# yweweler/single-speaker-tts

Measured on AMD Instinct MI355X. Metric: mel-frames/sec (end-to-end text->waveform incl. 60-iter Griffin-Lim, 64-utt LJ-Speech-shaped batch per GPU), higher is better.
Workload: dtype f32

## Files before the change

### single-speaker-tts_amd/csrc/api_internal.h

```cpp
#pragma once
#include <cmath>
#include <cstdio>
#include <cstring>
#include <memory>
#include <mutex>
#include <string>
#include <utility>
#include <vector>
#include "decoder.h"
#include "griffin_lim.h"
#include "tts_common.h"
#include <algorithm>
#include <map>

namespace tts_api {
using namespace tts;


extern thread_local std::string g_create_error;

struct ManifestEntry {
    std::string name;
    std::vector<int64_t> shape;
    size_t numel() const {
// ... 9 lines not shown
    const float* proj_wt[2];
    const float* proj_b[2];
    const float* proj_scale[2];
    const float* proj_shift[2];
    const float* lifter_wt;
    const float* lifter_b;
    std::vector<const float*> hw_wt, hw_b;
    const float* gru_in_wt;
    const float* gru_in_b;
    const float* gru_rec;
};

enum Stage { ST_ENCODER = 0, ST_DECODER, ST_POSTNET, ST_DENORM, ST_GL_ITER, ST_GL_FINAL, ST_DEBUG_GEMM, ST_EVAL_LOSS, ST_FEATURES, ST_COUNT };
extern const char* const kStageNames[ST_COUNT];

struct ProfSpan {
    hipEvent_t a, b;
    int stage;
    int64_t launches;
};


}
using namespace tts_api;

struct tts_handle_s {
    tts_config_t cfg;
    int device = 0;
    hipStream_t stream = nullptr;
    bool own_stream = false;
    std::string err;
    int use_graph = 0;
    int fused_tail = 1;
    bool tail_configured = false;
    int profile = 0;
    int pipeline = 1;
    int reserve_cus = 32;
    int hold_lds_kb = 64;
    hipStream_t aux = nullptr;
    int* hold_flags = nullptr;
    hipEvent_t ev_aux = nullptr;
    unsigned call_count = 0;
    hipStream_t front = nullptr;
    hipStream_t encs = nullptr;
    int enc_stream = 1;
    hipEvent_t ev_enc_ready[2] = {nullptr, nullptr};
    hipEvent_t ev_dec_done[2] = {nullptr, nullptr};
    hipEvent_t ev_gap[2] = {nullptr, nullptr};
    bool enc_ready_pending[2] = {false, false}, dec_done_pending[2] = {false, false}, gap_pending[2] = {false, false};
    hipEvent_t ev_front_done = nullptr;
    hipEvent_t ev_post_done[2] = {nullptr, nullptr};
    bool post_pending[2] = {false, false};
    bool gl_wide_used[2] = {false, false};
    hipEvent_t ev_gl_done[2] = {nullptr, nullptr};
    bool gl_pending[2] = {false, false};
    bool front_pending = false;
    hipEvent_t ev_serial_done = nullptr;
    bool serial_pending = false;
    unsigned syn_calls = 0;
    int syn_shape[3] = {0, 0, 0};
    int last_enc_ahead = -1;
    bool in_synthesize = false;
    int persistent_decoder = 1;
    int pd_ws = 1;
    bool ws_configured = false;
    int gl_pair = 3;
// ... 176 lines not shown
        if (!h->profile) return;
        ProfSpan s{};
        if (hipEventCreate(&s.a) != hipSuccess || hipEventCreate(&s.b) != hipSuccess) return;
        s.stage = stage;
        s.launches = launches;
        hipEventRecord(s.a, h->stream);
        h->spans.push_back(s);
        idx = (int)h->spans.size() - 1;
    }
    ~ProfScope() {
        if (idx >= 0) hipEventRecord(h->spans[idx].b, h->stream);
    }
};

struct SynthScope {
    tts_handle_t h;
    explicit SynthScope(tts_handle_t h_) : h(h_) { h->in_synthesize = true; }
    ~SynthScope() { h->in_synthesize = false; }
};

int fail(tts_handle_t h, int code, const std::string& msg);
void build_manifest(tts_handle_t h);
int check_status(tts_handle_t h);
int sync_all(tts_handle_t h);
int graph_quiesce(tts_handle_t h);
int graph_drop(tts_handle_t h);
int ws_get(tts_handle_t h, const char* name, size_t bytes, void** out);
void prof_collect(tts_handle_t h);
void feat_release(tts_handle_t h);
GemmGroup dense_group(const float* A, int lda, const float* Wt, const float* bias, float* C, int ldc, int M, int N, int K, int act);
GemmGroup conv_group(const float* A, int Cin, int ktaps, int T, const float* Wt, const float* bias, const float* scale, const float* shift, float* C, int ldc, int coff, int M, int N, int act, int pool);
int run_single(tts_handle_t h, const GemmGroup& g);
bool graph_runtime_ok(int* have);
int run_cbhg(tts_handle_t h, const CbhgWeights& w, const char* tag, const float* x, int B, int T, float* out, int64_t* launches);
int check_ready(tts_handle_t h);
int gl_tables(tts_handle_t h);
int device_cus(tts_handle_t h);
int stft_prepare(tts_handle_t h, int n, int win, int hop, int n_fft);
int stft_run(tts_handle_t h, const float* wav, int B, int n, int n_fft, int win, int hop, float2** out, int* Tf_out);
int gl_fp(int n_fft);
bool gl_is_streaming(int n_fft, int win, int hop);
int glg_twiddles(tts_handle_t h, int n_fft, const float2** out);
int glg_prepare(tts_handle_t h, int T, int win, int hop, int n_fft);
int gl_run_generic(tts_handle_t h, const float* mag_int, const float* init_ft, uint64_t seed, int B, int T, int n_iter, int win, int hop, int n_fft, float* wav, float* mse, bool peak_normalize);
int gl_prepare(tts_handle_t h, int T, int win, int hop, int n_fft);
int gl_run(tts_handle_t h, const float* mag_int, const float* init_ft, uint64_t seed, int B, int T, int n_iter, int win, int hop, int n_fft, float* wav, float* mse, bool peak_normalize = false, bool under_reservation = false, float2* const* phase_pair = nullptr, bool phase_ready = false, int wide_from = -1);
int standalone_begin(tts_handle_t h);
int standalone_end(tts_handle_t h);
int encoder_impl(tts_handle_t h, const int32_t* ids, int B, int Ts, float* memory);
int pd_kernel_for(tts_handle_t h, int B, int Ts, int budget);
int pd_choice(tts_handle_t h, int B, int Ts, int budget, bool pipelined);
int attention_keys(tts_handle_t h, const float* memory, int B, int Ts, float* keys);
int decoder_impl(tts_handle_t h, const float* memory, int B, int Ts, int n_steps, float* mel, float* alignments);
int postnet_impl(tts_handle_t h, const float* mel, int B, int T, float* linear, float* mag, float ref_db, float max_db, float power, int* db_flag = nullptr);
bool denorm_can_assert(float ref_db, float max_db);
int denorm_flag_arm(tts_handle_t h, int** flag);
int denorm_flag_read(tts_handle_t h);
int gl_wide_from(tts_handle_t h, int B, int Ts, int n_steps, int T, int n_iter);

}
```

### single-speaker-tts_amd/csrc/api_stages.hip

```cpp
#include "api_internal.h"

namespace tts_api {


int run_cbhg(tts_handle_t h, const CbhgWeights& w, const char* tag, const float* x, int B, int T, float* out,
             int64_t* launches) {
    const tts_config_t& c = h->cfg;
    const int M = B * T;
    const int NB = w.n_banks, NF = w.n_filters;
    const int U = c.n_highway_units, H = c.n_gru_units;
    const std::string t(tag);
    WS(h, (t + ".bank").c_str(), float, (size_t)M * NB * NF, bank);
    WS(h, (t + ".p1").c_str(), float, (size_t)M * w.proj_filters[0], p1);
    WS(h, (t + ".p2").c_str(), float, (size_t)M * w.proj_filters[1], p2);
    WS(h, (t + ".hw0").c_str(), float, (size_t)M * U, hw0);
    WS(h, (t + ".hw1").c_str(), float, (size_t)M * U, hw1);
    WS(h, (t + ".xproj").c_str(), float, (size_t)M * 6 * H, xproj);

    for (int k0 = 0; k0 < NB; k0 += TTS_GEMM_MAX_GROUPS) {
        GemmBatch b;
        std::memset(&b, 0, sizeof(b));
        const int ng = std::min(TTS_GEMM_MAX_GROUPS, NB - k0);
        for (int i = 0; i < ng; ++i) {
            const int k = k0 + ng - 1 - i;
            b.g[i] = conv_group(x, w.c_in, k + 1, T, w.bank_wt[k], w.bank_b[k], w.bank_scale[k], w.bank_shift[k], bank,
                                NB * NF, k * NF, M, NF, ACT_RELU, 0);
        }
        HIPCHK(h, launch_gemm(h->stream, b, ng));
        ++*launches;
    }
    {
        GemmGroup g = conv_group(bank, NB * NF, 3, T, w.proj_wt[0], w.proj_b[0], w.proj_scale[0], w.proj_shift[0], p1,
                                 w.proj_filters[0], 0, M, w.proj_filters[0], ACT_RELU, 1);
        const int slices = gemm_splitk_slices(g.K);
        if (slices > 1) {
            WS(h, (t + ".splitk").c_str(), float, (size_t)slices * M * g.N, part);
            HIPCHK(h, launch_gemm_splitk(h->stream, g, slices, part));
            ++*launches;
        } else {
            int rc = run_single(h, g);
            if (rc) return rc;
        }
        ++*launches;
    }
    {
        GemmGroup g = conv_group(p1, w.proj_filters[0], 3, T, w.proj_wt[1], w.proj_b[1], w.proj_scale[1],
                                 w.proj_shift[1], p2, w.proj_filters[1], 0, M, w.proj_filters[1], ACT_NONE, 0);
        g.R = x;
        g.ldr = w.c_in;
        int rc = run_single(h, g);
        if (rc) return rc;
        ++*launches;
    }
    if (h->fused_tail && cbhg_tail_supports(w.proj_filters[1], U, H, (int)w.hw_wt.size(), M)) {
        if (!h->tail_configured) {
            HIPCHK(h, cbhg_tail_configure());
            h->tail_configured = true;
        }
        CbhgTailParams tp;
        std::memset(&tp, 0, sizeof(tp));
        tp.X = p2; tp.ldx = w.proj_filters[1]; tp.c_in = w.proj_filters[1];
        tp.lifter_wt = w.lifter_wt; tp.lifter_b = w.lifter_b;
        tp.n_hw = (int)w.hw_wt.size();
        for (int l = 0; l < tp.n_hw; ++l) { tp.hw_wt[l] = w.hw_wt[l]; tp.hw_b[l] = w.hw_b[l]; }
        tp.gru_wt = w.gru_in_wt; tp.gru_b = w.gru_in_b;
        tp.hw_out = hw0; tp.xproj = xproj; tp.M = M;
        HIPCHK(h, launch_cbhg_tail(h->stream, tp));
        ++*launches;
    } else {
        {
            int rc = run_single(h, dense_group(p2, w.proj_filters[1], w.lifter_wt, w.lifter_b, hw0, U, M, U,
                                               w.proj_filters[1], ACT_RELU));
            if (rc) return rc;
            ++*launches;
        }
        float* cur = hw0;
        float* nxt = hw1;
        for (size_t l = 0; l < w.hw_wt.size(); ++l) {
            GemmGroup g = dense_group(cur, U, w.hw_wt[l], w.hw_b[l], nxt, U, M, 2 * U, U, ACT_NONE);
            g.epi = EPI_HIGHWAY;
            int rc = run_single(h, g);
            if (rc) return rc;
            ++*launches;
            std::swap(cur, nxt);
        }
        {
            int rc = run_single(h, dense_group(cur, U, w.gru_in_wt, w.gru_in_b, xproj, 6 * H, M, 6 * H, U, ACT_NONE));
            if (rc) return rc;
            ++*launches;
        }
    }
    HIPCHK(h, launch_bigru(h->stream, xproj, 6 * H, w.gru_rec, out, B, T, H, c.force_cudnn));
    ++*launches;
    return TTS_OK;
}


int check_ready(tts_handle_t h) {
    if (!h) return TTS_ERR_INVALID;
// ... 373 lines not shown
        if (h->dec_done_pending[i]) HIPCHK(h, hipStreamWaitEvent(h->stream, h->ev_dec_done[i], 0));
    }
    return TTS_OK;
}

int standalone_end(tts_handle_t h) {
    if (h->in_synthesize || !h->front) return TTS_OK;
    if (!h->ev_serial_done) HIPCHK(h, hipEventCreateWithFlags(&h->ev_serial_done, hipEventDisableTiming));
    HIPCHK(h, hipEventRecord(h->ev_serial_done, h->stream));
    h->serial_pending = true;
    return TTS_OK;
}

int encoder_impl(tts_handle_t h, const int32_t* ids, int B, int Ts, float* memory) {
    int rc = TTS_OK;
    const tts_config_t& c = h->cfg;
    const int M = B * Ts;
    WS(h, "enc.pre1", float, (size_t)M * c.enc_prenet_units[0], pre1);
    WS(h, "enc.pre2", float, (size_t)M * c.enc_prenet_units[1], pre2);
    int64_t launches = 0;
    ProfScope ps(h, ST_ENCODER, 0);
    {
        GemmGroup g = dense_group(h->embedding, c.embedding_size, h->enc_pre_wt[0], h->enc_pre_b[0], pre1,
                                  c.enc_prenet_units[0], M, c.enc_prenet_units[0], c.embedding_size, ACT_RELU);
        g.gather = ids;
        g.gather_rows = c.vocabulary_size;
        if ((rc = run_single(h, g))) return rc;
    }
    if ((rc = run_single(h, dense_group(pre1, c.enc_prenet_units[0], h->enc_pre_wt[1], h->enc_pre_b[1], pre2,
                                        c.enc_prenet_units[1], M, c.enc_prenet_units[1], c.enc_prenet_units[0],
                                        ACT_RELU))))
        return rc;
    launches += 2;
    if ((rc = run_cbhg(h, h->enc, "enc", pre2, B, Ts, memory, &launches))) return rc;
    if (ps.idx >= 0) h->spans[ps.idx].launches = launches;
    return TTS_OK;
}


int pd_kernel_for(tts_handle_t h, int B, int Ts, int budget) {
    const int cudnn = h->cfg.force_cudnn;
    if (h->pd_ws && decoder_ws_supports(h->dec, cudnn, B, Ts) && decoder_ws_workgroups(B) <= budget) return 2;
    if (decoder_persistent_supports(h->dec, cudnn, B, Ts) && decoder_persistent_workgroups(B) <= budget) return 1;
    return 0;
}


int pd_choice(tts_handle_t h, int B, int Ts, int budget, bool pipelined) {
    if (h->persistent_decoder <= 0) return 0;
    const int k = pd_kernel_for(h, B, Ts, budget);
    if (h->persistent_decoder >= 2) return k;
    if (k == 2) return 2;
    if (k == 1) return (pipelined && B > 48) ? 1 : 0;
    return 0;
}


int attention_keys(tts_handle_t h, const float* memory, int B, int Ts, float* keys) {
    const int A = h->cfg.n_attention_units, mem = 2 * h->cfg.n_gru_units;
    return run_single(h, dense_group(memory, mem, h->mem_wt, nullptr, keys, A, B * Ts, A, mem, ACT_NONE));
}

int decoder_impl(tts_handle_t h, const float* memory, int B, int Ts, int n_steps, float* mel, float* alignments) {
    int rc = TTS_OK;
    const tts_config_t& c = h->cfg;
    if (h->dec.local_d > 0 && Ts < 2 * h->dec.local_d + 1)
        return fail(h, TTS_ERR_UNSUPPORTED,
// ... 131 lines not shown
        if (defer_proj) {
            h->pending_proj = proj;
            h->has_pending_proj = true;
        } else if ((rc = run_single(h, proj))) {
            return rc;
        }
    }
    if (predictive) {
        int flag = 0;
        HIPCHK(h, hipMemcpyAsync(&flag, sc.err_flag, sizeof(int), hipMemcpyDeviceToHost, h->stream));
        HIPCHK(h, hipStreamSynchronize(h->stream));
        if (flag)
            return fail(h, TTS_ERR_UNSUPPORTED,
                        "LocalLuongAttention (predictive): a predicted attention window leaves the memory; the "
                        "reference pads such windows inconsistently and fails there too");
    }
    return TTS_OK;
}


int postnet_impl(tts_handle_t h, const float* mel, int B, int T, float* linear, float* mag, float ref_db,
                        float max_db, float power, int* db_flag) {
    int rc = check_ready(h);
    if (rc) return rc;
    if (!mel || (!linear && !mag) || B < 1 || T < 1) return fail(h, TTS_ERR_INVALID, "postnet_forward: bad arguments");
    const tts_config_t& c = h->cfg;
    const int M = B * T, H2 = 2 * c.n_gru_units, F = 1 + c.n_fft / 2;
    int64_t launches = 0;
    ProfScope ps(h, ST_POSTNET, 0);
    const float* dense_in = mel;
    int dense_k = c.n_mels;
    if (c.apply_post_processing) {
        WS(h, "post.gru", float, (size_t)M * H2, gru);
        if ((rc = run_cbhg(h, h->post, "post", mel, B, T, gru, &launches))) return rc;
        dense_in = gru;
        dense_k = H2;
    }
    GemmGroup g = dense_group(dense_in, dense_k, h->dense_wt, h->dense_b, linear, F, M, F, dense_k, ACT_NONE);
    if (mag) {
        g.C2 = mag;
        g.ldc2 = gl_fp(c.n_fft);
        g.N2 = gl_fp(c.n_fft);
        g.d_ref = ref_db;
        g.d_range = std::fabs(ref_db) + std::fabs(max_db);
        g.d_pow = power;
        g.d_flag = db_flag;
    }
    if ((rc = run_single(h, g))) return rc;
    ++launches;
    if (ps.idx >= 0) h->spans[ps.idx].launches = launches;
    return TTS_OK;
}


bool denorm_can_assert(float ref_db, float max_db) {
    return ref_db - (std::fabs(ref_db) + std::fabs(max_db)) < -100.0f;
}

int denorm_flag_arm(tts_handle_t h, int** flag) {
    if (!h->an.flag) HIPCHK(h, hipMalloc(&h->an.flag, sizeof(int)));
    HIPCHK(h, hipMemsetAsync(h->an.flag, 0, sizeof(int), h->stream));
    *flag = h->an.flag;
    return TTS_OK;
}

int denorm_flag_read(tts_handle_t h) {
    int flag = 0;
// ... 278 lines not shown
```

### single-speaker-tts_amd/csrc/cbhg_tail.hip

```cpp
#include "tts_common.h"

namespace tts {

#define CT_BM 128
#define CT_U 128
#define CT_XLD (CT_U + 4)
#define CT_BK 32
#define CT_BLD (CT_BK + 4)
#define CT_BN 256
#define CT_THREADS 512

#define CT_AIMG (3 * CT_BM * 64)
#define CT_BIMG (3 * CT_BN * 64)
size_t cbhg_tail_lds_bytes() { return (size_t)CT_BM * CT_XLD * sizeof(float) + CT_AIMG + CT_BIMG; }
typedef __bf16 ct_bf16x8_t __attribute__((ext_vector_type(8)));
__device__ __forceinline__ void ct_split3(float x, unsigned& h, unsigned& m, unsigned& l) {
    h = __float_as_uint(x);
    const float r1 = x - __uint_as_float(h & 0xFFFF0000u);
    m = __float_as_uint(r1);
    const float r2 = r1 - __uint_as_float(m & 0xFFFF0000u);
    l = __float_as_uint(r2);
}
__device__ __forceinline__ unsigned ct_pack_hi(unsigned a, unsigned b) { return __builtin_amdgcn_perm(b, a, 0x07060302u); }
__device__ __forceinline__ void ct_store_split4(unsigned char* img, int rows, int row, int kq, float4 v) {
    unsigned h[4], m[4], l[4];
    ct_split3(v.x, h[0], m[0], l[0]);
    ct_split3(v.y, h[1], m[1], l[1]);
    ct_split3(v.z, h[2], m[2], l[2]);
    ct_split3(v.w, h[3], m[3], l[3]);
    const int off = (row * 4 + ((kq >> 1) ^ ((row >> 2) & 3))) * 16 + (kq & 1) * 8;
    *reinterpret_cast<uint2*>(img + off) = make_uint2(ct_pack_hi(h[0], h[1]), ct_pack_hi(h[2], h[3]));
    *reinterpret_cast<uint2*>(img + rows * 64 + off) = make_uint2(ct_pack_hi(m[0], m[1]), ct_pack_hi(m[2], m[3]));
    *reinterpret_cast<uint2*>(img + 2 * rows * 64 + off) = make_uint2(ct_pack_hi(l[0], l[1]), ct_pack_hi(l[2], l[3]));
}

bool cbhg_tail_supports(int c_in, int units, int gru_units, int n_hw, long long M) {
    return units == CT_U && gru_units == 128 && c_in >= 4 && c_in <= CT_U && c_in % 4 == 0 && n_hw >= 0 && n_hw <= CBHG_TAIL_MAX_HW &&
           M >= 1 && (M + CT_BM) * 3 * CT_BN * (long long)sizeof(float) < 0xFFFFFFF0ll;
}

__global__ __launch_bounds__(CT_THREADS) void cbhg_tail_kernel(CbhgTailParams p) {
    extern __shared__ __attribute__((aligned(16))) float lds[];
    float* Xs = lds;
    unsigned char* Ai = reinterpret_cast<unsigned char*>(lds + CT_BM * CT_XLD);
    unsigned char* Bi = Ai + CT_AIMG;
    const int tid = threadIdx.x, lane = tid & 63, wave = tid >> 6;
    const int wm = wave & 1, wn = wave >> 1;
    const int li = lane & 31, lh = lane >> 5;
    const int m0 = blockIdx.x * CT_BM;
    const int M = p.M;

    {
        const __amdgpu_buffer_rsrc_t rs = __builtin_amdgcn_make_buffer_rsrc(const_cast<float*>(p.X), 0, (int)0xFFFFFFF0u, 0x00020000);
#pragma unroll
        for (int i = 0; i < (CT_BM * (CT_U / 4)) / CT_THREADS; ++i) {
            const int idx = tid + CT_THREADS * i;
            const int row = idx >> 5, c4 = idx & 31;
            const bool ok = m0 + row < M && 4 * c4 < p.c_in;
            const unsigned off = ok ? (unsigned)((size_t)(m0 + row) * p.ldx + 4 * c4) * 4u : 0xFFFFFFFFu;
            const float4 v = __builtin_bit_cast(float4, __builtin_amdgcn_raw_buffer_load_b128(rs, (int)off, 0, 0));
            *reinterpret_cast<float4*>(&Xs[row * CT_XLD + 4 * c4]) = v;
        }
    }

    const int n_jobs = 1 + p.n_hw + 3;
    const int kq = tid & 7;
    float4 rb[4];
    auto job_w = [&](int j) -> const float* {
        return j == 0 ? p.lifter_wt : (j <= p.n_hw ? p.hw_wt[j - 1] : p.gru_wt + (size_t)(j - 1 - p.n_hw) * CT_BN * CT_U);
    };
    auto job_k = [&](int j) { return j == 0 ? p.c_in : CT_U; };
    auto job_n = [&](int j) { return j == 0 ? CT_U : CT_BN; };
    auto load_chunk = [&](int j, int kc) {
        const __amdgpu_buffer_rsrc_t rs = __builtin_amdgcn_make_buffer_rsrc(const_cast<float*>(job_w(j)), 0, (int)0xFFFFFFF0u, 0x00020000);
        const int K = job_k(j), N = job_n(j);
        const int kk = kc * CT_BK + 4 * kq;
#pragma unroll
        for (int i = 0; i < 4; ++i) {
            const int row = (tid >> 3) + 64 * i;
            const bool ok = row < N && kk < K;
            rb[i] = __builtin_bit_cast(float4, __builtin_amdgcn_raw_buffer_load_b128(rs, ok ? (int)((unsigned)(row * K + kk) * 4u) : -1, 0, 0));
        }
    };
    auto stage_chunk = [&](int kc) {
#pragma unroll
        for (int i = 0; i < 4; ++i) ct_store_split4(Bi, CT_BN, (tid >> 3) + 64 * i, kq, rb[i]);
#pragma unroll
        for (int i = 0; i < 2; ++i) {
            const int row = (tid >> 3) + 64 * i;
            ct_store_split4(Ai, CT_BM, row, kq, *reinterpret_cast<const float4*>(&Xs[row * CT_XLD + kc * CT_BK + 4 * kq]));
        }
    };

    const __amdgpu_buffer_rsrc_t xp_rs = __builtin_amdgcn_make_buffer_rsrc(
        p.xproj, 0, (int)(unsigned)((size_t)M * 3 * CT_BN * sizeof(float) < 0xFFFFFFF0ull ? (size_t)M * 3 * CT_BN * sizeof(float) : 0xFFFFFFF0ull), 0x00020000);
    const __amdgpu_buffer_rsrc_t hw_rs = __builtin_amdgcn_make_buffer_rsrc(
        p.hw_out, 0, p.hw_out ? (int)(unsigned)((size_t)M * CT_U * sizeof(float)) : 0, 0x00020000);
    const int row_l = wm * 64 + 4 * lh;

    f32x16 acc[2][2];
    load_chunk(0, 0);
    for (int j = 0; j < n_jobs; ++j) {
        const int nch = (job_k(j) + CT_BK - 1) / CT_BK;
        const bool live = 64 * wn < job_n(j);
#pragma unroll
        for (int a = 0; a < 2; ++a)
#pragma unroll
            for (int b = 0; b < 2; ++b)
#pragma unroll
                for (int r = 0; r < 16; ++r) acc[a][b][r] = 0.f;
        for (int kc = 0; kc < nch; ++kc) {
            __syncthreads();
            stage_chunk(kc);
            __syncthreads();
            if (kc + 1 < nch) load_chunk(j, kc + 1);
            else if (j + 1 < n_jobs) load_chunk(j + 1, 0);
            if (live) {
#pragma unroll
                for (int q = 0; q < 2; ++q) {
                    const int ch = 2 * q + lh;
                    uint4 fa[2][3];
#pragma unroll
                    for (int tm = 0; tm < 2; ++tm) {
                        const int row = wm * 64 + tm * 32 + li;
                        const int off = (row * 4 + (ch ^ ((row >> 2) & 3))) * 16;
#pragma unroll
                        for (int sp = 0; sp < 3; ++sp) fa[tm][sp] = *reinterpret_cast<const uint4*>(Ai + sp * CT_BM * 64 + off);
                    }
#pragma unroll
                    for (int tn = 0; tn < 2; ++tn) {
                        const int row = wn * 64 + tn * 32 + li;
                        const int off = (row * 4 + (ch ^ ((row >> 2) & 3))) * 16;
                        uint4 fb[3];
#pragma unroll
                        for (int sp = 0; sp < 3; ++sp) fb[sp] = *reinterpret_cast<const uint4*>(Bi + sp * CT_BN * 64 + off);
#pragma unroll
                        for (int tm = 0; tm < 2; ++tm) {
#define CT_MMA(SA, SB)                                                                                                   \
                            acc[tm][tn] = __builtin_amdgcn_mfma_f32_32x32x16_bf16(__builtin_bit_cast(ct_bf16x8_t, fa[tm][SA]), \
                                                                                  __builtin_bit_cast(ct_bf16x8_t, fb[SB]), acc[tm][tn], 0, 0, 0);
                            CT_MMA(0, 2) CT_MMA(2, 0) CT_MMA(1, 1) CT_MMA(0, 1) CT_MMA(1, 0) CT_MMA(0, 0)
#undef CT_MMA
                        }
                    }
                }
            }
        }

        if (j == 0) {
            if (live) {
#pragma unroll
                for (int tn = 0; tn < 2; ++tn) {
                    const float b = p.lifter_b[wn * 64 + tn * 32 + li];
#pragma unroll
                    for (int tm = 0; tm < 2; ++tm)
#pragma unroll
                        for (int r = 0; r < 16; ++r) acc[tm][tn][r] = fmaxf(acc[tm][tn][r] + b, 0.f);
                }
            }
            __syncthreads();
            if (live) {
#pragma unroll
                for (int tn = 0; tn < 2; ++tn)
#pragma unroll
                    for (int tm = 0; tm < 2; ++tm)
#pragma unroll
                        for (int r = 0; r < 16; ++r) {
                            const int ro = tm * 32 + (r & 3) + 8 * (r >> 2);
                            Xs[(row_l + ro) * CT_XLD + wn * 64 + tn * 32 + li] = acc[tm][tn][r];
                        }
            }
        } else if (j <= p.n_hw) {
            const int unit = wn * 32 + li;
            const float bh = p.hw_b[j - 1][wn * 64 + li], bt = p.hw_b[j - 1][wn * 64 + 32 + li];
#pragma unroll
            for (int tm = 0; tm < 2; ++tm)
#pragma unroll
                for (int r = 0; r < 16; ++r) {
                    const int ro = tm * 32 + (r & 3) + 8 * (r >> 2);
                    const float hh = fmaxf(acc[tm][0][r] + bh, 0.f);
                    const float tt = sigmoidf_(acc[tm][1][r] + bt);
                    const float x = Xs[(row_l + ro) * CT_XLD + unit];
// ... 63 lines not shown
```

### single-speaker-tts_amd/csrc/tts_common.h

```cpp
#pragma once
#include <hip/hip_runtime.h>
#include <stdint.h>
#include <stddef.h>
#include <map>
#include <string>
#include <vector>

#include "../../include/sstts_hip.h"

namespace tts {

typedef float f32x4 __attribute__((ext_vector_type(4)));
typedef float f32x16 __attribute__((ext_vector_type(16)));

enum Act { ACT_NONE = 0, ACT_RELU = 1, ACT_SIGMOID = 2, ACT_TANH = 3 };
enum Epi { EPI_STD = 0, EPI_HIGHWAY = 1 };

__device__ __forceinline__ float sigmoidf_(float x) { return __builtin_amdgcn_rcpf(1.0f + __expf(-x)); }
__device__ __forceinline__ double wave_sum_f64(double v) {
#pragma unroll
    for (int o = 32; o > 0; o >>= 1) v += __shfl_xor(v, o);
    return v;
}
__device__ __forceinline__ void split_f64(double v, float* hi, float* lo) {
// ... 38 lines not shown
    const float* R;
    float* C;
    int M, N, K;
    int lda, T, Cin, padl, pool;
    int ldc, coff, ldr;
    int act, epi;
    float* C2;
    int ldc2, N2;
    float d_ref, d_range, d_pow;
    int* d_flag;
    int kt0, kt1;
};
#define TTS_GEMM_MAX_GROUPS 16
struct GemmBatch {
    GemmGroup g[TTS_GEMM_MAX_GROUPS];
};
hipError_t launch_gemm(hipStream_t s, const GemmBatch& b, int n_groups);
hipError_t launch_gemm_splitk(hipStream_t s, const GemmGroup& g, int slices, float* partial);
int gemm_splitk_slices(int K);

hipError_t launch_bigru(hipStream_t s, const float* xproj, int xld, const float* wrec, float* out,
                        int B, int T, int H, int cudnn);
size_t bigru_wrec_floats(int H, int cudnn);

#define CBHG_TAIL_MAX_HW 8
struct CbhgTailParams {
    const float* X; int ldx; int c_in;
    const float* lifter_wt; const float* lifter_b;
    const float* hw_wt[CBHG_TAIL_MAX_HW]; const float* hw_b[CBHG_TAIL_MAX_HW]; int n_hw;
    const float* gru_wt; const float* gru_b;
    float* hw_out;
    float* xproj;
    int M;
};
bool cbhg_tail_supports(int c_in, int units, int gru_units, int n_hw, long long M);
hipError_t cbhg_tail_configure();
hipError_t launch_cbhg_tail(hipStream_t s, const CbhgTailParams& p);

hipError_t cu_hold_configure();
hipError_t launch_cu_hold(hipStream_t s, int n_cus, const int* flag, double timeout_ms, int lds_kb = 64);

size_t eval_loss_partial_count(int B, int T, int n_mels, int F);
hipError_t launch_eval_loss(hipStream_t s, const float* mel_t, const float* mel_o, const float* lin_t, const float* lin_o, int B,
                            int T, int n_mels, int F, int max_blocks, double* partial, double* sums, float* losses);

struct DevBuf {
    void* p = nullptr;
    size_t bytes = 0;
};

}
```

### single-speaker-tts_amd/csrc/api_handle.hip

```cpp
#include "api_internal.h"

namespace tts_api {
thread_local std::string g_create_error;
const char* const kStageNames[ST_COUNT] = {"encoder", "decoder", "postnet", "denorm", "gl_iter", "gl_final", "debug_gemm", "eval_loss", "features"};
}

namespace tts_api {


int fail(tts_handle_t h, int code, const std::string& msg) {
    if (h) h->err = msg;
    else g_create_error = msg;
    return code;
}


const char* kAtt = "decoder2/decoder/output_projection_wrapper/multi_rnn_cell/cell_0/attention_wrapper";

const char* kMrc = "decoder2/decoder/output_projection_wrapper/multi_rnn_cell";


std::string bn_name(int i) {
    return i == 0 ? std::string("batch_normalization") : "batch_normalization_" + std::to_string(i);
}
// ... 621 lines not shown
    h->gl_pending[0] = h->gl_pending[1] = false;
    h->gl_wide_used[0] = h->gl_wide_used[1] = false;
    {
        int rc = graph_drop(h);
        if (rc) return rc;
    }
    if (h->own_stream) hipStreamDestroy(h->stream);
    if (s) {
        h->stream = reinterpret_cast<hipStream_t>(s);
        h->own_stream = false;
    } else {
        HIPCHK(h, hipStreamCreate(&h->stream));
        h->own_stream = true;
    }
    return TTS_OK;
}


int tts_set_option(tts_handle_t h, const char* key, int value) {
    DeviceScope dev_scope(h);
    if (!h || !key) return TTS_ERR_INVALID;
    if (!std::strcmp(key, "use_graph")) {
        int have = 0;
        if (value && !(value == 2 && h->debug_hooks) && !graph_runtime_ok(&have))
            return fail(h, TTS_ERR_UNSUPPORTED,
                        "use_graph: this process runs the library on HIP runtime " + std::to_string(have) + ", older than the " +
                        std::to_string(HIP_VERSION) + " it was built with (a libamdhip64 loaded before the library, e.g. the one "
                        "PyTorch bundles); hipGraph replays of the decoder are wrong there (csrc/api_internal.h, `use_graph`) -- the "
                        "launches are enqueued directly instead");
        h->use_graph = value;
    }
    else if (!std::strcmp(key, "profile")) h->profile = value;
    else if (!std::strcmp(key, "fused_tail")) h->fused_tail = value;
    else if (!std::strcmp(key, "persistent_decoder")) {
        if (value != h->persistent_decoder) {
            int rc = sync_all(h);
            if (rc) return rc;
        }
        h->persistent_decoder = value;
    }
    else if (!std::strcmp(key, "gl_pair")) h->gl_pair = value;
    else if (!std::strcmp(key, "gl_wide_from")) h->gl_wide = value < -2 ? -2 : value;
    else if (!std::strcmp(key, "pd_ws")) {
        if (value != h->pd_ws) {
            int rc = sync_all(h);
            if (rc) return rc;
        }
        h->pd_ws = value;
    }
    else if (!std::strcmp(key, "enc_stream")) {
        int rc = sync_all(h);
        if (rc) return rc;
        h->enc_stream = value;
    }
    else if (!std::strcmp(key, "debug_hooks")) h->debug_hooks = value;
    else if (!std::strcmp(key, "pd_debug_delay") || !std::strcmp(key, "gl_runs") || !std::strcmp(key, "gl_run_len") ||
             !std::strcmp(key, "timeline") || !std::strcmp(key, "gl_workers") || !std::strcmp(key, "pd_rows")) {
        if (!h->debug_hooks && value != 0)
            return fail(h, TTS_ERR_INVALID, std::string(key) + ": a test hook; set the option \"debug_hooks\" to 1 on this handle first");
        if (!std::strcmp(key, "pd_debug_delay")) h->pd_debug_delay = value;
        else if (!std::strcmp(key, "gl_runs")) h->gl_runs = value;
        else if (!std::strcmp(key, "gl_run_len")) h->gl_run_len = value;
        else if (!std::strcmp(key, "gl_workers")) h->gl_workers = value;
        else if (!std::strcmp(key, "pd_rows")) h->pd_rows = value;
        else h->timeline = value;
    }
// ... 327 lines not shown
```

Before: 4.391 million.

## Fold second CBHG projection conv and residual into fused tail kernel prologue

For the post-net CBHG, the second projection conv (3-tap over p1, with bias, batchnorm scale/shift and the residual add of the input) is computed inside the fused tail kernel as an extra GEMM job that writes straight into shared memory. This removes one kernel launch and the global write and re-read of the p2 intermediate. The encoder keeps the old path via keep_p2. The tail kernel becomes more complex and gains extra registers, and the prologue loads p1 rows per tap through buffer loads.

```diff
diff --git a/single-speaker-tts_amd/csrc/api_internal.h b/single-speaker-tts_amd/csrc/api_internal.h
--- a/single-speaker-tts_amd/csrc/api_internal.h
+++ b/single-speaker-tts_amd/csrc/api_internal.h
@@ -307,7 +307,8 @@
 GemmGroup conv_group(const float* A, int Cin, int ktaps, int T, const float* Wt, const float* bias, const float* scale, const float* shift, float* C, int ldc, int coff, int M, int N, int act, int pool);
 int run_single(tts_handle_t h, const GemmGroup& g);
 bool graph_runtime_ok(int* have);
-int run_cbhg(tts_handle_t h, const CbhgWeights& w, const char* tag, const float* x, int B, int T, float* out, int64_t* launches);
+int run_cbhg(tts_handle_t h, const CbhgWeights& w, const char* tag, const float* x, int B, int T, float* out, int64_t* launches,
+             bool keep_p2);
 int check_ready(tts_handle_t h);
 int gl_tables(tts_handle_t h);
 int device_cus(tts_handle_t h);
diff --git a/single-speaker-tts_amd/csrc/api_stages.hip b/single-speaker-tts_amd/csrc/api_stages.hip
--- a/single-speaker-tts_amd/csrc/api_stages.hip
+++ b/single-speaker-tts_amd/csrc/api_stages.hip
@@ -4,7 +4,7 @@
 
 
 int run_cbhg(tts_handle_t h, const CbhgWeights& w, const char* tag, const float* x, int B, int T, float* out,
-             int64_t* launches) {
+             int64_t* launches, bool keep_p2) {
     const tts_config_t& c = h->cfg;
     const int M = B * T;
     const int NB = w.n_banks, NF = w.n_filters;
@@ -43,7 +43,9 @@
         }
         ++*launches;
     }
-    {
+    const bool tail = h->fused_tail && cbhg_tail_supports(w.proj_filters[1], U, H, (int)w.hw_wt.size(), M);
+    const bool fold = tail && h->fused_tail != 2 && !keep_p2 && cbhg_tail_prologue_supports(w.proj_filters[0], w.proj_filters[1], M);
+    if (!fold) {
         GemmGroup g = conv_group(p1, w.proj_filters[0], 3, T, w.proj_wt[1], w.proj_b[1], w.proj_scale[1],
                                  w.proj_shift[1], p2, w.proj_filters[1], 0, M, w.proj_filters[1], ACT_NONE, 0);
         g.R = x;
@@ -52,7 +54,7 @@
         if (rc) return rc;
         ++*launches;
     }
-    if (h->fused_tail && cbhg_tail_supports(w.proj_filters[1], U, H, (int)w.hw_wt.size(), M)) {
+    if (tail) {
         if (!h->tail_configured) {
             HIPCHK(h, cbhg_tail_configure());
             h->tail_configured = true;
@@ -65,6 +67,12 @@
         for (int l = 0; l < tp.n_hw; ++l) { tp.hw_wt[l] = w.hw_wt[l]; tp.hw_b[l] = w.hw_b[l]; }
         tp.gru_wt = w.gru_in_wt; tp.gru_b = w.gru_in_b;
         tp.hw_out = hw0; tp.xproj = xproj; tp.M = M;
+        if (fold) {
+            tp.X = nullptr;
+            tp.p1 = p1; tp.p1_c = w.proj_filters[0]; tp.T = T;
+            tp.p2_wt = w.proj_wt[1]; tp.p2_b = w.proj_b[1]; tp.p2_scale = w.proj_scale[1]; tp.p2_shift = w.proj_shift[1];
+            tp.R = x; tp.ldr = w.c_in;
+        }
         HIPCHK(h, launch_cbhg_tail(h->stream, tp));
         ++*launches;
     } else {
@@ -504,7 +512,7 @@
                                         ACT_RELU))))
         return rc;
     launches += 2;
-    if ((rc = run_cbhg(h, h->enc, "enc", pre2, B, Ts, memory, &launches))) return rc;
+    if ((rc = run_cbhg(h, h->enc, "enc", pre2, B, Ts, memory, &launches, true))) return rc;
     if (ps.idx >= 0) h->spans[ps.idx].launches = launches;
     return TTS_OK;
 }
@@ -702,7 +710,7 @@
     int dense_k = c.n_mels;
     if (c.apply_post_processing) {
         WS(h, "post.gru", float, (size_t)M * H2, gru);
-        if ((rc = run_cbhg(h, h->post, "post", mel, B, T, gru, &launches))) return rc;
+        if ((rc = run_cbhg(h, h->post, "post", mel, B, T, gru, &launches, false))) return rc;
         dense_in = gru;
         dense_k = H2;
     }
diff --git a/single-speaker-tts_amd/csrc/cbhg_tail.hip b/single-speaker-tts_amd/csrc/cbhg_tail.hip
--- a/single-speaker-tts_amd/csrc/cbhg_tail.hip
+++ b/single-speaker-tts_amd/csrc/cbhg_tail.hip
@@ -34,6 +34,12 @@
     *reinterpret_cast<uint2*>(img + 2 * rows * 64 + off) = make_uint2(ct_pack_hi(l[0], l[1]), ct_pack_hi(l[2], l[3]));
 }
 
+bool cbhg_tail_prologue_supports(int p1_c, int c_in, long long M) {
+    return p1_c >= CT_BK && p1_c % CT_BK == 0 && c_in >= 4 && c_in <= CT_U && c_in % 4 == 0 &&
+           (M + CT_BM) * p1_c * (long long)sizeof(float) < 0xFFFFFFF0ll && (M + CT_BM) * CT_U * (long long)sizeof(float) < 0xFFFFFFF0ll &&
+           (long long)c_in * 3 * p1_c * (long long)sizeof(float) < 0xFFFFFFF0ll;
+}
+
 bool cbhg_tail_supports(int c_in, int units, int gru_units, int n_hw, long long M) {
     return units == CT_U && gru_units == 128 && c_in >= 4 && c_in <= CT_U && c_in % 4 == 0 && n_hw >= 0 && n_hw <= CBHG_TAIL_MAX_HW &&
            M >= 1 && (M + CT_BM) * 3 * CT_BN * (long long)sizeof(float) < 0xFFFFFFF0ll;
@@ -50,7 +56,8 @@
     const int m0 = blockIdx.x * CT_BM;
     const int M = p.M;
 
-    {
+    const bool pro = p.p1 != nullptr;
+    if (!pro) {
         const __amdgpu_buffer_rsrc_t rs = __builtin_amdgcn_make_buffer_rsrc(const_cast<float*>(p.X), 0, (int)0xFFFFFFF0u, 0x00020000);
 #pragma unroll
         for (int i = 0; i < (CT_BM * (CT_U / 4)) / CT_THREADS; ++i) {
@@ -63,32 +70,59 @@
         }
     }
 
+    const int j_first = pro ? -1 : 0;
     const int n_jobs = 1 + p.n_hw + 3;
     const int kq = tid & 7;
     float4 rb[4];
+    float4 ra[2];
     auto job_w = [&](int j) -> const float* {
-        return j == 0 ? p.lifter_wt : (j <= p.n_hw ? p.hw_wt[j - 1] : p.gru_wt + (size_t)(j - 1 - p.n_hw) * CT_BN * CT_U);
+        return j < 0 ? p.p2_wt : j == 0 ? p.lifter_wt : (j <= p.n_hw ? p.hw_wt[j - 1] : p.gru_wt + (size_t)(j - 1 - p.n_hw) * CT_BN * CT_U);
     };
-    auto job_k = [&](int j) { return j == 0 ? p.c_in : CT_U; };
-    auto job_n = [&](int j) { return j == 0 ? CT_U : CT_BN; };
+    auto job_k = [&](int j) { return j < 0 ? 3 * p.p1_c : j == 0 ? p.c_in : CT_U; };
+    auto job_n = [&](int j) { return j < 0 ? p.c_in : j == 0 ? CT_U : CT_BN; };
+    int pro_t[2] = {-1, -1};
+    if (pro) {
+#pragma unroll
+        for (int i = 0; i < 2; ++i) {
+            const int m = m0 + (tid >> 3) + 64 * i;
+            pro_t[i] = m < M ? m % p.T : -1;
+        }
+    }
+    auto chunk_k0 = [&](int j, int kc) { return j < 0 ? (kc % 3) * p.p1_c + (kc / 3) * CT_BK : kc * CT_BK; };
     auto load_chunk = [&](int j, int kc) {
         const __amdgpu_buffer_rsrc_t rs = __builtin_amdgcn_make_buffer_rsrc(const_cast<float*>(job_w(j)), 0, (int)0xFFFFFFF0u, 0x00020000);
         const int K = job_k(j), N = job_n(j);
-        const int kk = kc * CT_BK + 4 * kq;
+        const int kk = chunk_k0(j, kc) + 4 * kq;
 #pragma unroll
         for (int i = 0; i < 4; ++i) {
+            if (i >= 2 && N <= 128) break;
             const int row = (tid >> 3) + 64 * i;
             const bool ok = row < N && kk < K;
             rb[i] = __builtin_bit_cast(float4, __builtin_amdgcn_raw_buffer_load_b128(rs, ok ? (int)((unsigned)(row * K + kk) * 4u) : -1, 0, 0));
         }
+        if (j < 0) {
+            const __amdgpu_buffer_rsrc_t ps = __builtin_amdgcn_make_buffer_rsrc(const_cast<float*>(p.p1), 0, (int)0xFFFFFFF0u, 0x00020000);
+            const int tap = kc % 3, ch = (kc / 3) * CT_BK + 4 * kq;
+#pragma unroll
+            for (int i = 0; i < 2; ++i) {
+                const int ts = pro_t[i] - 1 + tap;
+                const bool ok = pro_t[i] >= 0 && ts >= 0 && ts < p.T;
+                const int src = m0 + (tid >> 3) + 64 * i - 1 + tap;
+                ra[i] = __builtin_bit_cast(float4, __builtin_amdgcn_raw_buffer_load_b128(
+                                                       ps, ok ? (int)((unsigned)(src * p.p1_c + ch) * 4u) : -1, 0, 0));
+            }
+        }
     };
-    auto stage_chunk = [&](int kc) {
-#pragma unroll
-        for (int i = 0; i < 4; ++i) ct_store_split4(Bi, CT_BN, (tid >> 3) + 64 * i, kq, rb[i]);
+    auto stage_chunk = [&](int j, int kc) {
+#pragma unroll
+        for (int i = 0; i < 4; ++i) {
+            if (i >= 2 && job_n(j) <= 128) break;
+            ct_store_split4(Bi, CT_BN, (tid >> 3) + 64 * i, kq, rb[i]);
+        }
 #pragma unroll
         for (int i = 0; i < 2; ++i) {
             const int row = (tid >> 3) + 64 * i;
-            ct_store_split4(Ai, CT_BM, row, kq, *reinterpret_cast<const float4*>(&Xs[row * CT_XLD + kc * CT_BK + 4 * kq]));
+            ct_store_split4(Ai, CT_BM, row, kq, j < 0 ? ra[i] : *reinterpret_cast<const float4*>(&Xs[row * CT_XLD + kc * CT_BK + 4 * kq]));
         }
     };
 
@@ -99,8 +133,8 @@
     const int row_l = wm * 64 + 4 * lh;
 
     f32x16 acc[2][2];
-    load_chunk(0, 0);
-    for (int j = 0; j < n_jobs; ++j) {
+    load_chunk(j_first, 0);
+    for (int j = j_first; j < n_jobs; ++j) {
         const int nch = (job_k(j) + CT_BK - 1) / CT_BK;
         const bool live = 64 * wn < job_n(j);
 #pragma unroll
@@ -111,7 +145,7 @@
                 for (int r = 0; r < 16; ++r) acc[a][b][r] = 0.f;
         for (int kc = 0; kc < nch; ++kc) {
             __syncthreads();
-            stage_chunk(kc);
+            stage_chunk(j, kc);
             __syncthreads();
             if (kc + 1 < nch) load_chunk(j, kc + 1);
             else if (j + 1 < n_jobs) load_chunk(j + 1, 0);
@@ -147,7 +181,41 @@
             }
         }
 
-        if (j == 0) {
+        if (j < 0) {
+            if (live) {
+#pragma unroll
+                for (int tn = 0; tn < 2; ++tn) {
+                    const int c = wn * 64 + tn * 32 + li;
+                    const bool cok = c < p.c_in;
+                    const float b = cok ? p.p2_b[c] : 0.f;
+                    const float sc = cok && p.p2_scale ? p.p2_scale[c] : 1.f;
+                    const float sh = cok && p.p2_scale ? p.p2_shift[c] : 0.f;
+#pragma unroll
+                    for (int tm = 0; tm < 2; ++tm)
+#pragma unroll
+                        for (int r = 0; r < 16; ++r) {
+                            const int ro = tm * 32 + (r & 3) + 8 * (r >> 2);
+                            float v = acc[tm][tn][r] + b;
+                            v = v * sc + sh;
+                            Xs[(row_l + ro) * CT_XLD + c] = v;
+                        }
+                }
+            }
+            __syncthreads();
+            const __amdgpu_buffer_rsrc_t rs = __builtin_amdgcn_make_buffer_rsrc(const_cast<float*>(p.R), 0, (int)0xFFFFFFF0u, 0x00020000);
+#pragma unroll 1
+            for (int i = 0; i < (CT_BM * (CT_U / 4)) / CT_THREADS; ++i) {
+                const int idx = tid + CT_THREADS * i;
+                const int row = idx >> 5, c4 = idx & 31;
+                const bool ok = m0 + row < M && 4 * c4 < p.c_in;
+                const unsigned off = ok ? (unsigned)((size_t)(m0 + row) * p.ldr + 4 * c4) * 4u : 0xFFFFFFFFu;
+                const float4 x = __builtin_bit_cast(float4, __builtin_amdgcn_raw_buffer_load_b128(rs, (int)off, 0, 0));
+                float4 v = *reinterpret_cast<const float4*>(&Xs[row * CT_XLD + 4 * c4]);
+                v = ok ? make_float4(v.x + x.x, v.y + x.y, v.z + x.z, v.w + x.w) : make_float4(0.f, 0.f, 0.f, 0.f);
+                *reinterpret_cast<float4*>(&Xs[row * CT_XLD + 4 * c4]) = v;
+                if (ok && p.p2_out) *reinterpret_cast<float4*>(&p.p2_out[(size_t)(m0 + row) * p.c_in + 4 * c4]) = v;
+            }
+        } else if (j == 0) {
             if (live) {
 #pragma unroll
                 for (int tn = 0; tn < 2; ++tn) {
diff --git a/single-speaker-tts_amd/csrc/tts_common.h b/single-speaker-tts_amd/csrc/tts_common.h
--- a/single-speaker-tts_amd/csrc/tts_common.h
+++ b/single-speaker-tts_amd/csrc/tts_common.h
@@ -94,7 +94,13 @@
     float* hw_out;
     float* xproj;
     int M;
+    const float* p1; int p1_c; int T;
+    const float* p2_wt; const float* p2_b;
+    const float* p2_scale; const float* p2_shift;
+    const float* R; int ldr;
+    float* p2_out;
 };
+bool cbhg_tail_prologue_supports(int p1_c, int c_in, long long M);
 bool cbhg_tail_supports(int c_in, int units, int gru_units, int n_hw, long long M);
 hipError_t cbhg_tail_configure();
 hipError_t launch_cbhg_tail(hipStream_t s, const CbhgTailParams& p);
```

Result: no change. 4.422 million, median of 6 (+0.7%).

## Fold second CBHG projection conv into fused post-net tail kernel

Applied to the files above, without the earlier changes.

For the post-net CBHG, the second projection conv1d (3-tap, with batchnorm scale/shift and residual add) is computed inside the fused cbhg_tail kernel. It uses split-bf16 MFMA over tiles of p1 staged in LDS, and the result goes straight into the kernel's LDS input tile. This removes one GEMM launch and the global round-trip of the p2 buffer. In exchange the tail kernel gets more code, more register pressure and extra synchronisation, and each block recomputes the conv for its own rows. The path is enabled by default behind the fold_proj2 option.

```diff
diff --git a/single-speaker-tts_amd/csrc/api_handle.hip b/single-speaker-tts_amd/csrc/api_handle.hip
--- a/single-speaker-tts_amd/csrc/api_handle.hip
+++ b/single-speaker-tts_amd/csrc/api_handle.hip
@@ -677,6 +677,7 @@
     }
     else if (!std::strcmp(key, "profile")) h->profile = value;
     else if (!std::strcmp(key, "fused_tail")) h->fused_tail = value;
+    else if (!std::strcmp(key, "fold_proj2")) h->fold_proj2 = value;
     else if (!std::strcmp(key, "persistent_decoder")) {
         if (value != h->persistent_decoder) {
             int rc = sync_all(h);
diff --git a/single-speaker-tts_amd/csrc/api_internal.h b/single-speaker-tts_amd/csrc/api_internal.h
--- a/single-speaker-tts_amd/csrc/api_internal.h
+++ b/single-speaker-tts_amd/csrc/api_internal.h
@@ -65,6 +65,7 @@
     std::string err;
     int use_graph = 0;
     int fused_tail = 1;
+    int fold_proj2 = 1;
     bool tail_configured = false;
     int profile = 0;
     int pipeline = 1;
diff --git a/single-speaker-tts_amd/csrc/api_stages.hip b/single-speaker-tts_amd/csrc/api_stages.hip
--- a/single-speaker-tts_amd/csrc/api_stages.hip
+++ b/single-speaker-tts_amd/csrc/api_stages.hip
@@ -43,7 +43,10 @@
         }
         ++*launches;
     }
-    {
+    const bool tail = h->fused_tail && cbhg_tail_supports(w.proj_filters[1], U, H, (int)w.hw_wt.size(), M);
+    const bool fold = tail && t == "post" && h->fold_proj2 && w.proj_filters[1] == w.c_in &&
+                      cbhg_tail_fold_supports(w.proj_filters[0], w.proj_filters[1], M);
+    if (!fold) {
         GemmGroup g = conv_group(p1, w.proj_filters[0], 3, T, w.proj_wt[1], w.proj_b[1], w.proj_scale[1],
                                  w.proj_shift[1], p2, w.proj_filters[1], 0, M, w.proj_filters[1], ACT_NONE, 0);
         g.R = x;
@@ -52,7 +55,7 @@
         if (rc) return rc;
         ++*launches;
     }
-    if (h->fused_tail && cbhg_tail_supports(w.proj_filters[1], U, H, (int)w.hw_wt.size(), M)) {
+    if (tail) {
         if (!h->tail_configured) {
             HIPCHK(h, cbhg_tail_configure());
             h->tail_configured = true;
@@ -65,6 +68,12 @@
         for (int l = 0; l < tp.n_hw; ++l) { tp.hw_wt[l] = w.hw_wt[l]; tp.hw_b[l] = w.hw_b[l]; }
         tp.gru_wt = w.gru_in_wt; tp.gru_b = w.gru_in_b;
         tp.hw_out = hw0; tp.xproj = xproj; tp.M = M;
+        if (fold) {
+            tp.X = nullptr;
+            tp.p1 = p1; tp.p2_cin = w.proj_filters[0]; tp.T = T;
+            tp.p2_wt = w.proj_wt[1]; tp.p2_b = w.proj_b[1]; tp.p2_scale = w.proj_scale[1]; tp.p2_shift = w.proj_shift[1];
+            tp.res = x;
+        }
         HIPCHK(h, launch_cbhg_tail(h->stream, tp));
         ++*launches;
     } else {
diff --git a/single-speaker-tts_amd/csrc/cbhg_tail.hip b/single-speaker-tts_amd/csrc/cbhg_tail.hip
--- a/single-speaker-tts_amd/csrc/cbhg_tail.hip
+++ b/single-speaker-tts_amd/csrc/cbhg_tail.hip
@@ -38,6 +38,10 @@
     return units == CT_U && gru_units == 128 && c_in >= 4 && c_in <= CT_U && c_in % 4 == 0 && n_hw >= 0 && n_hw <= CBHG_TAIL_MAX_HW &&
            M >= 1 && (M + CT_BM) * 3 * CT_BN * (long long)sizeof(float) < 0xFFFFFFF0ll;
 }
+bool cbhg_tail_fold_supports(int p2_cin, int c_in, long long M) {
+    return p2_cin >= CT_BK && p2_cin % CT_BK == 0 && c_in <= 3 * 32 && (M + 1) * p2_cin * (long long)sizeof(float) < 0xFFFFFFF0ll &&
+           (long long)c_in * 3 * p2_cin * (long long)sizeof(float) < 0xFFFFFFF0ll;
+}
 
 __global__ __launch_bounds__(CT_THREADS) void cbhg_tail_kernel(CbhgTailParams p) {
     extern __shared__ __attribute__((aligned(16))) float lds[];
@@ -50,7 +54,8 @@
     const int m0 = blockIdx.x * CT_BM;
     const int M = p.M;
 
-    {
+    const bool fold = p.p2_wt != nullptr;
+    if (!fold) {
         const __amdgpu_buffer_rsrc_t rs = __builtin_amdgcn_make_buffer_rsrc(const_cast<float*>(p.X), 0, (int)0xFFFFFFF0u, 0x00020000);
 #pragma unroll
         for (int i = 0; i < (CT_BM * (CT_U / 4)) / CT_THREADS; ++i) {
@@ -66,6 +71,20 @@
     const int n_jobs = 1 + p.n_hw + 3;
     const int kq = tid & 7;
     float4 rb[4];
+    unsigned p1_taps[2] = {0u, 0u};
+    int p1_row[2] = {0, 0};
+    if (fold) {
+#pragma unroll
+        for (int i = 0; i < 2; ++i) {
+            const int m = m0 + (tid >> 3) + 64 * i;
+            const int t = m < M ? m % p.T : 0;
+            unsigned bits = 0;
+            for (int tap = 0; tap < 3; ++tap)
+                if (m < M && t - 1 + tap >= 0 && t - 1 + tap < p.T) bits |= 1u << tap;
+            p1_taps[i] = bits;
+            p1_row[i] = m - 1;
+        }
+    }
     auto job_w = [&](int j) -> const float* {
         return j == 0 ? p.lifter_wt : (j <= p.n_hw ? p.hw_wt[j - 1] : p.gru_wt + (size_t)(j - 1 - p.n_hw) * CT_BN * CT_U);
     };
@@ -91,6 +110,28 @@
             ct_store_split4(Ai, CT_BM, row, kq, *reinterpret_cast<const float4*>(&Xs[row * CT_XLD + kc * CT_BK + 4 * kq]));
         }
     };
+    auto p2_load = [&](int kc, float4* a, float4* w) {
+        const int tap = kc % 3, cb = (kc / 3) * CT_BK + 4 * kq;
+        const int kk = tap * p.p2_cin + cb, K = 3 * p.p2_cin;
+        const __amdgpu_buffer_rsrc_t ars = __builtin_amdgcn_make_buffer_rsrc(const_cast<float*>(p.p1), 0, (int)0xFFFFFFF0u, 0x00020000);
+        const __amdgpu_buffer_rsrc_t wrs = __builtin_amdgcn_make_buffer_rsrc(const_cast<float*>(p.p2_wt), 0, (int)0xFFFFFFF0u, 0x00020000);
+#pragma unroll
+        for (int i = 0; i < 2; ++i) {
+            const bool ok = (p1_taps[i] >> tap) & 1u;
+            a[i] = __builtin_bit_cast(float4, __builtin_amdgcn_raw_buffer_load_b128(
+                ars, ok ? (int)((unsigned)((p1_row[i] + tap) * p.p2_cin + cb) * 4u) : -1, 0, 0));
+            const int row = (tid >> 3) + 64 * i;
+            w[i] = __builtin_bit_cast(float4, __builtin_amdgcn_raw_buffer_load_b128(wrs, row < p.c_in ? (int)((unsigned)(row * K + kk) * 4u) : -1, 0, 0));
+        }
+    };
+    auto p2_stage = [&](const float4* a, const float4* w) {
+#pragma unroll
+        for (int i = 0; i < 2; ++i) {
+            const int row = (tid >> 3) + 64 * i;
+            ct_store_split4(Bi, CT_BN, row, kq, w[i]);
+            ct_store_split4(Ai, CT_BM, row, kq, a[i]);
+        }
+    };
 
     const __amdgpu_buffer_rsrc_t xp_rs = __builtin_amdgcn_make_buffer_rsrc(
         p.xproj, 0, (int)(unsigned)((size_t)M * 3 * CT_BN * sizeof(float) < 0xFFFFFFF0ull ? (size_t)M * 3 * CT_BN * sizeof(float) : 0xFFFFFFF0ull), 0x00020000);
@@ -99,7 +140,79 @@
     const int row_l = wm * 64 + 4 * lh;
 
     f32x16 acc[2][2];
-    load_chunk(0, 0);
+    if (fold) {
+        const int nch = 3 * p.p2_cin / CT_BK;
+#pragma unroll
+        for (int b = 0; b < 2; ++b)
+#pragma unroll
+            for (int r = 0; r < 16; ++r) acc[0][b][r] = 0.f;
+        auto p2_mma = [&]() {
+            const int rbk = wave & 3, cb0 = wave < 4 ? 0 : 2;
+#pragma unroll
+            for (int q = 0; q < 2; ++q) {
+                const int ch = 2 * q + lh;
+                uint4 fa[3];
+                {
+                    const int row = rbk * 32 + li;
+                    const int off = (row * 4 + (ch ^ ((row >> 2) & 3))) * 16;
+#pragma unroll
+                    for (int sp = 0; sp < 3; ++sp) fa[sp] = *reinterpret_cast<const uint4*>(Ai + sp * CT_BM * 64 + off);
+                }
+#pragma unroll
+                for (int tn = 0; tn < 2; ++tn) {
+                    if (tn == 1 && wave >= 4) continue;
+                    const int row = (cb0 + tn) * 32 + li;
+                    const int off = (row * 4 + (ch ^ ((row >> 2) & 3))) * 16;
+                    uint4 fb[3];
+#pragma unroll
+                    for (int sp = 0; sp < 3; ++sp) fb[sp] = *reinterpret_cast<const uint4*>(Bi + sp * CT_BN * 64 + off);
+#define CT_MMA(SA, SB)                                                                                                   \
+                    acc[0][tn] = __builtin_amdgcn_mfma_f32_32x32x16_bf16(__builtin_bit_cast(ct_bf16x8_t, fa[SA]),     \
+                                                                         __builtin_bit_cast(ct_bf16x8_t, fb[SB]), acc[0][tn], 0, 0, 0);
+                    CT_MMA(0, 2) CT_MMA(2, 0) CT_MMA(1, 1) CT_MMA(0, 1) CT_MMA(1, 0) CT_MMA(0, 0)
+#undef CT_MMA
+                }
+            }
+        };
+        float4 a0[2], w0[2], a1[2], w1[2];
+        p2_load(0, a0, w0);
+        if (nch > 1) p2_load(1, a1, w1);
+        for (int kc = 0; kc < nch; kc += 2) {
+            __syncthreads();
+            p2_stage(a0, w0);
+            __syncthreads();
+            if (kc + 2 < nch) p2_load(kc + 2, a0, w0);
+            else if (kc + 1 >= nch) load_chunk(0, 0);
+            p2_mma();
+            if (kc + 1 < nch) {
+                __syncthreads();
+                p2_stage(a1, w1);
+                __syncthreads();
+                if (kc + 3 < nch) p2_load(kc + 3, a1, w1);
+                else if (kc + 2 >= nch) load_chunk(0, 0);
+                p2_mma();
+            }
+        }
+        const int rbk = wave & 3, cb0 = wave < 4 ? 0 : 2;
+#pragma unroll
+        for (int tn = 0; tn < 2; ++tn) {
+            if (tn == 1 && wave >= 4) continue;
+            const int n = (cb0 + tn) * 32 + li;
+            const bool nok = n < p.c_in;
+            const float bv = nok ? p.p2_b[n] : 0.f, sc = nok ? p.p2_scale[n] : 1.f, sh = nok ? p.p2_shift[n] : 0.f;
+#pragma unroll
+            for (int r = 0; r < 16; ++r) {
+                const int ro = rbk * 32 + (r & 3) + 8 * (r >> 2) + 4 * lh;
+                const bool ok = nok && m0 + ro < M;
+                float v = acc[0][tn][r] + bv;
+                v = v * sc + sh;
+                if (ok) v += p.res[(size_t)(m0 + ro) * p.c_in + n];
+                Xs[ro * CT_XLD + n] = ok ? v : 0.f;
+            }
+        }
+    } else {
+        load_chunk(0, 0);
+    }
     for (int j = 0; j < n_jobs; ++j) {
         const int nch = (job_k(j) + CT_BK - 1) / CT_BK;
         const bool live = 64 * wn < job_n(j);
diff --git a/single-speaker-tts_amd/csrc/tts_common.h b/single-speaker-tts_amd/csrc/tts_common.h
--- a/single-speaker-tts_amd/csrc/tts_common.h
+++ b/single-speaker-tts_amd/csrc/tts_common.h
@@ -94,8 +94,12 @@
     float* hw_out;
     float* xproj;
     int M;
+    const float* p1; int p2_cin; int T;
+    const float* p2_wt; const float* p2_b; const float* p2_scale; const float* p2_shift;
+    const float* res;
 };
 bool cbhg_tail_supports(int c_in, int units, int gru_units, int n_hw, long long M);
+bool cbhg_tail_fold_supports(int p2_cin, int c_in, long long M);
 hipError_t cbhg_tail_configure();
 hipError_t launch_cbhg_tail(hipStream_t s, const CbhgTailParams& p);
 
```

After: 4.403 million before, 4.421 million after (median of 6 runs). No clear change (+0.4%).
